# pvjosue/CWFA

Measured on AMD Instinct MI355X. Metric: volumes/sec inverse-pass @512×512×96 fp32; NLL match vs ref (1/2/4/8 GPU), higher is better.
Workload: dtype f32 (storage, accumulation, wavelets, couplings); convolution products on the bf16 matrix cores from an exact three-way bf16 split of both fp32 operands, six products per fp32 product: fp32-equivalent; plain-fp32-MFMA figure: fp32_mfma; 1 GPU; 512x512x96 volume, 4-scale CWFA (CAT blocks, 64 ch) + LRNN inverse, z=0, batch 1/GPU, random-init weights (BASELINE.json configs[2]); precision=split, parallelism=replicated x1 (independent volumes per GPU, no collective)

## Files before the change

cwfa_amd/build.py:

```python
import os
import subprocess
import sys
from concurrent.futures import ThreadPoolExecutor

HERE = os.path.dirname(os.path.abspath(__file__))
CSRC = os.path.join(HERE, "csrc")
INCLUDE = os.path.join(os.path.dirname(HERE), "include")
LIB = os.path.join(HERE, "libcwfa_hip.so")
SOURCES = ["elementwise.hip", "conv2d.hip", "conv_wino.hip", "conv_wino2d.hip", "conv_split_layer.hip", "conv_split_out.hip", "conv_split3x3.hip", "conv3d.hip", "conv3d_split.hip", "lrnn_ops.hip", "conv_bwd.hip", "eval_ops.hip", "prep_ops.hip", "optim_ops.hip", "loss_ops.hip", "deconv_ops.hip", "neuron_ops.hip", "noise_ops.hip", "sparse_ops.hip", "register_ops.hip", "register_views_ops.hip", "register3d_ops.hip", "footprint_ops.hip", "trace_ops.hip", "demix_ops.hip"]
HIPCC = os.environ.get("HIPCC", "/opt/rocm/bin/hipcc")
FLAGS = ["--offload-arch=gfx950", "-O3", "-fPIC", "-std=c++17", "-ffp-contract=off", "-I", INCLUDE, "-I", CSRC,
         "-Wall", "-Wno-unused-function"]


EXTRA = {"conv3d_split.hip": ["-fno-slp-vectorize"], "demix_ops.hip": ["-ffp-contract=off"]}


def _newer(src, dst):
    return not os.path.exists(dst) or os.path.getmtime(src) > os.path.getmtime(dst)


def build_all(force=False, verbose=False):
    deps = [os.path.join(CSRC, "common.h"), os.path.join(CSRC, "conv_internal.h"), os.path.join(CSRC, "conv_split_out_geom.h"), os.path.join(CSRC, "register_internal.h"), os.path.join(INCLUDE, "cwfa_hip.h"),
            os.path.abspath(__file__)]
    objs, jobs = [], []
    for s in SOURCES:
        src, obj = os.path.join(CSRC, s), os.path.join(CSRC, s.replace(".hip", ".o"))
        objs.append(obj)
        if force or _newer(src, obj) or any(_newer(d, obj) for d in deps):
            jobs.append([HIPCC, *FLAGS, *EXTRA.get(s, []), "-c", src, "-o", obj])

    def run(cmd):
        if verbose:
            print(" ".join(cmd), flush=True)
        r = subprocess.run(cmd, capture_output=True, text=True)
        if r.returncode != 0:
            raise RuntimeError(f"hipcc failed: {' '.join(cmd)}\n{r.stdout}\n{r.stderr}")
        return r.stderr

    with ThreadPoolExecutor(max_workers=4) as ex:
        for warn in ex.map(run, jobs):
            if verbose and warn.strip():
                print(warn, file=sys.stderr)
    if jobs or force or not os.path.exists(LIB) or any(_newer(o, LIB) for o in objs):
        run([HIPCC, "--offload-arch=gfx950", "-shared", "-fPIC", "-o", LIB, *objs])
    return LIB


if __name__ == "__main__":
    print(build_all(force="--force" in sys.argv, verbose=True))
```

cwfa_amd/csrc/conv2d.hip:

```cpp
#include "conv_internal.h"

#include <string.h>
#include <type_traits>

namespace {

template <int KS_, int CK_, int MT_, int NT_, int WM_, int WN_, int XV_ = 1>
struct Cfg {
    static constexpr int KS = KS_, CK = CK_, MT = MT_, NT = NT_, WM = WM_, WN = WN_;
    static constexpr int XV = XV_;
    static_assert(XV_ == 1 || (XV_ == 4 && KS_ == 1), "vector staging needs halo-free tiles");
    static constexpr int PAD = KS / 2;
    static constexpr int NTHREADS = 64 * WM * WN;
    static constexpr int CT = 32 * MT * WM;
    static constexpr int TR = NT * WN;
    static constexpr int TC = 32;
    static constexpr int XR = TR + KS - 1;
    static constexpr int XC = TC + KS - 1;
    static constexpr int XS = CK * XR * XC;
    static constexpr int XS_PAD = (XS + 3) & ~3;
    static constexpr int WS = KS * KS * CK * CT;
    static constexpr int XPT = (XS / XV + NTHREADS - 1) / NTHREADS;
    static constexpr int WPT = (WS / 4 + NTHREADS - 1) / NTHREADS;
    static constexpr int BUF = XS_PAD + WS;
// ... 521 lines not shown
    if (rc) return rc;
    hipLaunchKernelGGL((conv2d_mfma_kernel<C, EPI, PRO>), grid, dim3(C::NTHREADS), LDS, stream, p);
    CWFA_LAUNCH_CHECK("cwfa_conv2d_f32");
    return CWFA_OK;
}

template <class C, unsigned ALLOWED, bool PRO>
int launch_sel(const ConvParams& p, int epi, hipStream_t st) {
    if (!(ALLOWED & (1u << epi)) && epi != EPI_NONE_BLK8) epi = EPI_GENERIC;
    switch (epi) {
        case EPI_NONE: if constexpr (ALLOWED & (1u << EPI_NONE)) return launch_epi<C, EPI_NONE, PRO>(p, st); break;
        case EPI_ELU: if constexpr (ALLOWED & (1u << EPI_ELU)) return launch_epi<C, EPI_ELU, PRO>(p, st); break;
        case EPI_RES_ELU: if constexpr (ALLOWED & (1u << EPI_RES_ELU)) return launch_epi<C, EPI_RES_ELU, PRO>(p, st); break;
        case EPI_PRELU: if constexpr (ALLOWED & (1u << EPI_PRELU)) return launch_epi<C, EPI_PRELU, PRO>(p, st); break;
        case EPI_RES_PRELU: if constexpr (ALLOWED & (1u << EPI_RES_PRELU)) return launch_epi<C, EPI_RES_PRELU, PRO>(p, st); break;
        case EPI_GELU_RES: if constexpr (ALLOWED & (1u << EPI_GELU_RES)) return launch_epi<C, EPI_GELU_RES, PRO>(p, st); break;
        case EPI_UP: if constexpr (ALLOWED & (1u << EPI_UP)) return launch_epi<C, EPI_UP, PRO>(p, st); break;
        case EPI_NONE_BLK8:
            if constexpr (ALLOWED & (1u << EPI_NONE_BLK8)) return launch_epi<C, EPI_NONE_BLK8, PRO>(p, st);
            cwfa_set_error("cwfa_conv2d_f32: out_blocked8 is built for the 1x1 kernels with more than 32 output channels");
            return CWFA_E_SHAPE;
        default: break;
    }
    return launch_epi<C, EPI_GENERIC, PRO>(p, st);
}

template <class C, unsigned ALLOWED, unsigned ALLOWED_PRO>
int launch(const ConvParams& p, int epi, hipStream_t st) {
    if (p.o.in_scale || p.o.in_add) return launch_sel<C, ALLOWED_PRO, true>(p, epi, st);
    return launch_sel<C, ALLOWED, false>(p, epi, st);
}

}
int g_cwfa_split_xcd_map = 1;
int g_cwfa_split_rows16 = 1;
extern int g_cwfa_mip3_ablate;
extern int g_cwfa_reg_upsample_stages;
namespace {

int fill_params(ConvParams& p, const char* name, const float* x, const float* w_packed, float* y, int B, int Cin, int H,
                int W, int Cout, int64_t x_bs, int64_t y_bs, const cwfa_conv_opts* opts) {
    CWFA_REQUIRE(B >= 0 && Cin > 0 && Cout > 0 && H >= 0 && W >= 0, CWFA_E_INVAL, "%s: bad size", name);
    if (B == 0 || H == 0 || W == 0) return 1;
    CWFA_REQUIRE(x && w_packed && y, CWFA_E_INVAL, "%s: null pointer", name);
    CWFA_REQUIRE(!opts || !opts->out_sample_stats, CWFA_E_INVAL, "%s: out_sample_stats is a feature of the few-channel cwfa_conv7x7_split_f32", name);
    CWFA_REQUIRE((int64_t)Cin * H * W < (1ll << 30) && (int64_t)Cout * H * W * (p.o.upshuffle2 ? 1 : 1) < (1ll << 30), CWFA_E_SHAPE, "%s: C*H*W exceeds the 32-bit byte offsets of a tile (2^30 elements per image)", name);
    CWFA_REQUIRE(cwfa_aligned16(w_packed), CWFA_E_ALIGN, "%s: packed weights must be 16-byte aligned", name);
    p.x = x; p.wp = w_packed; p.y = y;
    p.B = B; p.Cin = Cin; p.H = H; p.W = W; p.Cout = Cout;
    p.x_bs = x_bs; p.y_bs = y_bs;
    p.products = g_cwfa_operand == CwfaOperand::split3 ? 6 : 1;
    if (opts) p.o = *opts;
    CWFA_REQUIRE(!(p.o.in_scale && !p.o.in_shift), CWFA_E_INVAL, "%s: in_scale without in_shift", name);
    CWFA_REQUIRE(p.o.act >= 0 && p.o.act <= CWFA_ACT_RELU && p.o.act2 >= 0 && p.o.act2 <= CWFA_ACT_RELU, CWFA_E_INVAL,
                 "%s: bad activation", name);
    CWFA_REQUIRE(!((p.o.act == CWFA_ACT_PRELU || p.o.act2 == CWFA_ACT_PRELU) && !p.o.prelu_alpha), CWFA_E_INVAL,
                 "%s: PReLU without prelu_alpha", name);
    return CWFA_OK;
}

typedef Cfg<1, 16, 2, 4, 4, 2> CS;
constexpr int CS_XB = 3 * 2 * 8 * 32 * 16, CS_WB = 3 * 2 * 256 * 16, CS_BUFB = CS_XB + CS_WB;

__device__ __forceinline__ void split3(float v, unsigned short (&o)[3]) {
    const __bf16 a1 = (__bf16)v;
    const float r1 = v - (float)a1;
    const __bf16 a2 = (__bf16)r1;
    const float r2 = r1 - (float)a2;
    const __bf16 a3 = (__bf16)r2;
    o[0] = __builtin_bit_cast(unsigned short, a1);
    o[1] = __builtin_bit_cast(unsigned short, a2);
    o[2] = __builtin_bit_cast(unsigned short, a3);
}

__device__ __forceinline__ unsigned short f16_bits(float v) { return __builtin_bit_cast(unsigned short, (_Float16)v); }

template <bool F16 = false>
__global__ __launch_bounds__(256) void split_input_kernel(const float* __restrict__ x, uint4* __restrict__ ws, int Cin, int CG2,
                                                          int64_t HW, int64_t x_bs, const float* __restrict__ sc,
                                                          const float* __restrict__ sh, int64_t aff_bs,
                                                          const float* __restrict__ add, int64_t add_bs) {
    const int64_t px = (int64_t)blockIdx.x * 256 + threadIdx.x;
    if (px >= HW) return;
    const int cg = blockIdx.y, b = blockIdx.z;
    unsigned short pc[3][8];
#pragma unroll
    for (int j = 0; j < 8; ++j) {
        const int c = cg * 8 + j;
        float v = 0.f;
        if (c < Cin) {
            v = x[(int64_t)b * x_bs + (int64_t)c * HW + px];
            if (sc) v = v * sc[(int64_t)b * aff_bs + c] + sh[(int64_t)b * aff_bs + c];
            if (add) v += add[(int64_t)b * add_bs + (int64_t)c * HW + px];
        }
        if constexpr (F16) {
            pc[0][j] = f16_bits(v);
            continue;
        }
        unsigned short o[3];
        split3(v, o);
        pc[0][j] = o[0]; pc[1][j] = o[1]; pc[2][j] = o[2];
    }
#pragma unroll
    for (int q = 0; q < (F16 ? 1 : 3); ++q) {
        uint4 u;
        u.x = pc[q][0] | ((unsigned)pc[q][1] << 16);
        u.y = pc[q][2] | ((unsigned)pc[q][3] << 16);
        u.z = pc[q][4] | ((unsigned)pc[q][5] << 16);
        u.w = pc[q][6] | ((unsigned)pc[q][7] << 16);
        ws[(((int64_t)b * 3 + q) * CG2 + cg) * HW + px] = u;
    }
}

template <bool F16 = false>
__global__ __launch_bounds__(256) void split_pack_kernel(const float* __restrict__ w, uint4* __restrict__ out, int Cout, int Cin,
                                                         int nchunks, int taps, int transposed, int64_t total) {
    const int64_t i = (int64_t)blockIdx.x * blockDim.x + threadIdx.x;
    if (i >= total) return;
    const int col = (int)(i % 256), h = (int)((i / 256) % 2), tap = (int)((i / 512) % taps);
    const int chunk = (int)((i / (512 * (int64_t)taps)) % nchunks);
    const int ctile = (int)(i / ((int64_t)512 * taps * nchunks));
    const int co = ctile * 256 + col;
    unsigned short pc[3][8];
#pragma unroll
    for (int j = 0; j < 8; ++j) {
        const int ci = chunk * 16 + h * 8 + j;
        float v = 0.f;
        if (co < Cout && ci < Cin)
            v = transposed ? w[((int64_t)ci * (Cout / 4) + (co >> 2)) * 4 + (co & 3)] : w[((int64_t)co * Cin + ci) * taps + tap];
        if constexpr (F16) {
            pc[0][j] = f16_bits(v);
            pc[1][j] = pc[2][j] = 0;
            continue;
        }
        unsigned short o[3];
        split3(v, o);
        pc[0][j] = o[0]; pc[1][j] = o[1]; pc[2][j] = o[2];
    }
#pragma unroll
    for (int q = 0; q < 3; ++q) {
        uint4 u;
        u.x = pc[q][0] | ((unsigned)pc[q][1] << 16);
        u.y = pc[q][2] | ((unsigned)pc[q][3] << 16);
        u.z = pc[q][4] | ((unsigned)pc[q][5] << 16);
        u.w = pc[q][6] | ((unsigned)pc[q][7] << 16);
        out[((((int64_t)ctile * nchunks + chunk) * taps + tap) * 3 + q) * 512 + h * 256 + col] = u;
    }
}

struct SplitParams {
    ConvParams c;
    const void* ws;
    int CG2;
    int64_t ws_bs;
};

template <int EPI, bool F16 = false>
__global__ __launch_bounds__(512, 1) void conv1x1_split_kernel(SplitParams sp) {
    typedef CS C;
    const ConvParams& p = sp.c;
    extern __shared__ __attribute__((aligned(16))) float smem[];
    char* lds = reinterpret_cast<char*>(smem);
    const Tile t = make_tile<C>(p);
    const bool six = p.products != 1;
    const int tid = threadIdx.x, wave = tid >> 6;
    const int64_t HW = (int64_t)p.H * p.W;
    constexpr unsigned OOB = 0x80000000u;

    unsigned xoff[3];
#pragma unroll
    for (int i = 0; i < 3; ++i) {
        const int e = tid + i * 512;
        const int px = e & 31, row = (e >> 5) & 7, h = (e >> 8) & 1, piece = e >> 9;
        const int gr = t.row0 + row, gc = t.col0 + px;
        xoff[i] = (gr < p.H && gc < p.W) ? (unsigned)((((int64_t)piece * sp.CG2 + h) * HW + (int64_t)gr * p.W + gc) * 16) : OOB;
    }
    const auto rx = CWFA_RSRC(reinterpret_cast<const char*>(sp.ws) + (int64_t)t.b * sp.ws_bs, (int)sp.ws_bs);
    const auto rw = CWFA_RSRC(reinterpret_cast<const char*>(p.wp) + (int64_t)t.ct * p.nchunks * CS_WB, p.nchunks * CS_WB);
    const int xchunk = (int)(2 * HW * 16);
    constexpr int NPC = F16 ? 1 : 3;
    auto dma = [&](int chunk, int buf) {
        char* base = lds + buf * CS_BUFB + wave * 1024;
#pragma unroll
        for (int i = 0; i < NPC; ++i)
            __builtin_amdgcn_raw_ptr_buffer_load_lds(rx, (lds_ptr)(base + i * 8192), 16, xoff[i], chunk * xchunk, 0, 0);
#pragma unroll
        for (int i = 0; i < NPC; ++i)
            __builtin_amdgcn_raw_ptr_buffer_load_lds(rw, (lds_ptr)(base + CS_XB + i * 8192), 16, (unsigned)(tid + i * 512) * 16u,
                                                     chunk * CS_WB, 0, 0);
    };

    f32x16 acc[2][4];
#pragma unroll
    for (int m = 0; m < 2; ++m)
#pragma unroll
        for (int n = 0; n < 4; ++n)
#pragma unroll
            for (int r = 0; r < 16; ++r) acc[m][n][r] = 0.f;

    const char* alane = lds + CS_XB + ((t.kh * 256) + t.wm * 64 + t.l31) * 16;
    const char* blane = lds + ((t.kh * 8 + t.wn * 4) * 32 + t.l31) * 16;

    dma(0, 0);
    dma(1, 1);
    if constexpr (F16) asm volatile("s_waitcnt vmcnt(2)" ::: "memory");
    else asm volatile("s_waitcnt vmcnt(6)" ::: "memory");
    __builtin_amdgcn_s_barrier();
    int buf = 0;
    for (int chunk = 0; chunk < p.nchunks; ++chunk) {
        int nb = buf + 2;
        nb = nb >= 3 ? nb - 3 : nb;
        dma(chunk + 2, nb);
        const char* ab = alane + buf * CS_BUFB;
        const char* bb = blane + buf * CS_BUFB;
        bf16x8 A[2][3], Bq[2][3];
#pragma unroll
        for (int m = 0; m < 2; ++m)
#pragma unroll
            for (int q = 0; q < 3; ++q) A[m][q] = *reinterpret_cast<const bf16x8*>(ab + (q * 512 + m * 32) * 16);
#pragma unroll
        for (int q = 0; q < 3; ++q) Bq[0][q] = *reinterpret_cast<const bf16x8*>(bb + (q * 512) * 16);
#pragma unroll
        for (int n = 0; n < 4; ++n) {
            if (n < 3) {
#pragma unroll
                for (int q = 0; q < 3; ++q) Bq[(n + 1) & 1][q] = *reinterpret_cast<const bf16x8*>(bb + (q * 512 + (n + 1) * 32) * 16);
            }
#pragma unroll
            for (int m = 0; m < 2; ++m) {
                f32x16 c = acc[m][n];
                if constexpr (F16) {
                    acc[m][n] = __builtin_amdgcn_mfma_f32_32x32x16_f16(__builtin_bit_cast(f16x8, A[m][0]), __builtin_bit_cast(f16x8, Bq[n & 1][0]),
                                                                       c, 0, 0, 0);
                    continue;
                }
                if (six) {
                    c = __builtin_amdgcn_mfma_f32_32x32x16_bf16(A[m][2], Bq[n & 1][0], c, 0, 0, 0);
                    c = __builtin_amdgcn_mfma_f32_32x32x16_bf16(A[m][1], Bq[n & 1][1], c, 0, 0, 0);
                    c = __builtin_amdgcn_mfma_f32_32x32x16_bf16(A[m][0], Bq[n & 1][2], c, 0, 0, 0);
                    c = __builtin_amdgcn_mfma_f32_32x32x16_bf16(A[m][1], Bq[n & 1][0], c, 0, 0, 0);
                    c = __builtin_amdgcn_mfma_f32_32x32x16_bf16(A[m][0], Bq[n & 1][1], c, 0, 0, 0);
                }
                c = __builtin_amdgcn_mfma_f32_32x32x16_bf16(A[m][0], Bq[n & 1][0], c, 0, 0, 0);
                acc[m][n] = c;
            }
        }
        if constexpr (F16) asm volatile("s_waitcnt vmcnt(2)\n\ts_waitcnt lgkmcnt(0)" ::: "memory");
        else asm volatile("s_waitcnt vmcnt(6)\n\ts_waitcnt lgkmcnt(0)" ::: "memory");
        __builtin_amdgcn_s_barrier();
        buf = buf + 1 == 3 ? 0 : buf + 1;
    }
    asm volatile("s_waitcnt vmcnt(0)" ::: "memory");
    __syncthreads();
    epilogue<C, EPI>(p, t, acc);
}

template <int EPI>
int launch_split(SplitParams sp, hipStream_t stream) {
    ConvParams& p = sp.c;
    p.tiles_x = (p.W + CS::TC - 1) / CS::TC;
    p.tiles_y = (p.H + CS::TR - 1) / CS::TR;
    const int ctiles = (p.Cout + CS::CT - 1) / CS::CT;
    CWFA_REQUIRE((int64_t)p.tiles_x * p.tiles_y < (1ll << 31) && ctiles <= 65535 && p.B <= 65535, CWFA_E_SHAPE,
                 "cwfa_conv_split_f32: grid too large");
    constexpr int LDS = 3 * CS_BUFB;
    return cwfa_with_operand([&](auto, auto f16) -> int {
        constexpr auto kern = &conv1x1_split_kernel<EPI, f16>;
        const int rc = cwfa_max_lds<kern>(LDS, "cwfa_conv_split_f32");
        if (rc) return rc;
        hipLaunchKernelGGL(kern, dim3((unsigned)(p.tiles_x * p.tiles_y), ctiles, p.B), dim3(512), LDS, stream, sp);
        CWFA_LAUNCH_CHECK("cwfa_conv_split_f32");
        return CWFA_OK;
    });
}

}

extern "C" int64_t cwfa_split_workspace_bytes(int B, int Cin, int64_t HW) {
    if (B < 0 || Cin <= 0 || HW < 0) return -1;
    const int64_t CG2 = 2 * ((Cin + 15) / 16);
    return (int64_t)B * 3 * CG2 * HW * 16;
}

extern "C" int cwfa_split_input_f32(const float* x, void* ws, int B, int Cin, int64_t HW, int64_t x_bs, const float* in_scale,
                                    const float* in_shift, int64_t in_affine_bs, const float* in_add, int64_t in_add_bs,
                                    void* stream) {
    CWFA_REQUIRE(x && ws, CWFA_E_INVAL, "cwfa_split_input_f32: null pointer");
    CWFA_REQUIRE(B >= 0 && Cin > 0 && HW >= 0 && B <= 65535, CWFA_E_SHAPE, "cwfa_split_input_f32: bad shape");
    CWFA_REQUIRE(!in_scale == !in_shift, CWFA_E_INVAL, "cwfa_split_input_f32: in_scale and in_shift go together");
    CWFA_REQUIRE(cwfa_aligned16(ws), CWFA_E_ALIGN, "cwfa_split_input_f32: workspace must be 16-byte aligned");
    if (B == 0 || HW == 0) return CWFA_OK;
    const int CG2 = 2 * ((Cin + 15) / 16);
    CWFA_REQUIRE((int64_t)3 * CG2 * HW * 16 < (1ll << 31), CWFA_E_SHAPE, "cwfa_split_input_f32: one sample's planes must stay below 2 GiB");
    return cwfa_with_operand([&](auto, auto f16) -> int {
        hipLaunchKernelGGL(split_input_kernel<f16>, dim3((unsigned)((HW + 255) / 256), CG2, B), dim3(256), 0, (hipStream_t)stream, x,
                           reinterpret_cast<uint4*>(ws), Cin, CG2, HW, x_bs, in_scale, in_shift, in_affine_bs, in_add, in_add_bs);
        CWFA_LAUNCH_CHECK("cwfa_split_input_f32");
        return CWFA_OK;
    });
}

extern "C" int64_t cwfa_conv_split_packed_bytes(int Cout, int Cin, int ks) {
    if (Cout <= 0 || Cin <= 0 || ks != 1) return -1;
    return (int64_t)((Cout + 255) / 256) * ((Cin + 15) / 16) * CS_WB;
}

extern "C" int cwfa_conv_split_pack_f32(const float* w, void* packed, int Cout, int Cin, int ks, int transposed, void* stream) {
    CWFA_REQUIRE(w && packed, CWFA_E_INVAL, "cwfa_conv_split_pack_f32: null pointer");
    CWFA_REQUIRE(Cout > 0 && Cin > 0 && ks == 1 && (!transposed || Cout % 4 == 0), CWFA_E_SHAPE,
                 "cwfa_conv_split_pack_f32: bad shape (1x1 / transposed 2x2 only; 3x3: cwfa_conv3x3_split_pack_f32)");
    CWFA_REQUIRE(cwfa_aligned16(packed), CWFA_E_ALIGN, "cwfa_conv_split_pack_f32: packed image must be 16-byte aligned");
    const int nchunks = (Cin + 15) / 16, taps = ks * ks;
    const int64_t total = (int64_t)((Cout + 255) / 256) * nchunks * taps * 512;
    return cwfa_with_operand([&](auto, auto f16) -> int {
        hipLaunchKernelGGL(split_pack_kernel<f16>, dim3((unsigned)((total + 255) / 256)), dim3(256), 0, (hipStream_t)stream, w,
                           reinterpret_cast<uint4*>(packed), Cout, Cin, nchunks, taps, transposed, total);
        CWFA_LAUNCH_CHECK("cwfa_conv_split_pack_f32");
        return CWFA_OK;
    });
}

extern "C" int cwfa_conv_split_f32(const void* ws, const void* w_packed, float* y, int B, int Cin, int H, int W, int Cout, int ks,
                                   int64_t y_bs, const cwfa_conv_opts* opts, void* stream) {
    CWFA_REQUIRE(!(opts && (opts->in_blocked8 || opts->out_blocked8 || opts->in_cat)), CWFA_E_INVAL,
                 "cwfa_conv_split_f32: blocked layouts / two-source inputs are not built here");
    CWFA_REQUIRE(ws && w_packed && y, CWFA_E_INVAL, "cwfa_conv_split_f32: null pointer");
    CWFA_REQUIRE(ks == 1, CWFA_E_SHAPE, "cwfa_conv_split_f32: kernel size %d (1x1 only; 3x3: cwfa_conv3x3_split_f32)", ks);
    SplitParams sp{};
    int rc = fill_params(sp.c, "cwfa_conv_split_f32", reinterpret_cast<const float*>(ws), reinterpret_cast<const float*>(w_packed), y,
                         B, Cin, H, W, Cout, 0, y_bs, opts);
    if (rc) return rc < 0 ? rc : CWFA_OK;
    ConvParams& p = sp.c;
    CWFA_REQUIRE(!p.o.in_scale && !p.o.in_add, CWFA_E_INVAL, "cwfa_conv_split_f32: the load-side prologue belongs in cwfa_split_input_f32");
    CWFA_REQUIRE(!p.o.upshuffle2 || (ks == 1 && Cout % 4 == 0), CWFA_E_SHAPE, "cwfa_conv_split_f32: upshuffle2 needs ks=1, Cout=4*Co");
    CWFA_REQUIRE(!p.o.out_stats && !p.o.prelu_per_channel, CWFA_E_INVAL, "cwfa_conv_split_f32: out_stats / prelu_per_channel are features of cwfa_conv3x3_split_f32");
    p.nchunks = (Cin + 15) / 16;
    sp.ws = ws;
    sp.CG2 = 2 * p.nchunks;
    sp.ws_bs = (int64_t)3 * sp.CG2 * H * W * 16;
    CWFA_REQUIRE(sp.ws_bs + (int64_t)4 * H * W * 16 < (1ll << 31) && (int64_t)(p.nchunks * ks * ks + 2) * CS_WB < (1ll << 31), CWFA_E_SHAPE,
                 "cwfa_conv_split_f32: one sample's planes / one cout tile's weights must stay below 2 GiB");
    const int epi = classify_epilogue(p.o);
    hipStream_t st = (hipStream_t)stream;
    switch (epi) {
        case EPI_NONE: return launch_split<EPI_NONE>(sp, st);
        case EPI_UP: return launch_split<EPI_UP>(sp, st);
        default: return launch_split<EPI_GENERIC>(sp, st);
    }
}

int g_cwfa_wino_min_cout = 1;
int g_cwfa_wino_2d = 512;
CwfaOperand g_cwfa_operand = CwfaOperand::split3;

extern "C" int cwfa_set_option(const char* name, int value) {
    CWFA_REQUIRE(name, CWFA_E_INVAL, "cwfa_set_option: null name");
    if (strcmp(name, "winograd_min_cout") == 0) {
        g_cwfa_wino_min_cout = value;
        return CWFA_OK;
    }
    if (strcmp(name, "winograd_2d") == 0) {
        g_cwfa_wino_2d = value;
        return CWFA_OK;
    }
    if (strcmp(name, "wgrad_split") == 0) {
        g_cwfa_wgrad_split = value != 0;
        return CWFA_OK;
    }
    if (strcmp(name, "wgrad_rows") == 0) {
        g_cwfa_wgrad_rows = value;
        return CWFA_OK;
    }
    if (strcmp(name, "split3x3_xcd_map") == 0) {
        g_cwfa_split_xcd_map = value;
        return CWFA_OK;
    }
    if (strcmp(name, "mip3_ablate") == 0) {
        CWFA_REQUIRE(value >= 0 && value <= 7, CWFA_E_INVAL, "cwfa_set_option: mip3_ablate is a mask of bits 0..2");
        g_cwfa_mip3_ablate = value;
        return CWFA_OK;
    }
    if (strcmp(name, "reg_upsample_stages") == 0) {
        CWFA_REQUIRE(value >= 0 && value <= 7, CWFA_E_INVAL, "cwfa_set_option: reg_upsample_stages is a mask of bits 0..2");
        g_cwfa_reg_upsample_stages = value;
        return CWFA_OK;
    }
    if (strcmp(name, "split3x3_rows16") == 0) {
        g_cwfa_split_rows16 = value;
        return CWFA_OK;
    }
    if (strcmp(name, "split_products") == 0) {
        CWFA_REQUIRE(value == 1 || value == 6, CWFA_E_INVAL, "cwfa_set_option: split_products must be 1 or 6");
        CWFA_REQUIRE(value == 1 || g_cwfa_operand != CwfaOperand::fp16, CWFA_E_INVAL,
                     "cwfa_set_option: split_products = 6 needs split_operand = 0 (the three-piece split is a bf16 format)");
        if (value == 6) g_cwfa_operand = CwfaOperand::split3;
        else if (g_cwfa_operand == CwfaOperand::split3) g_cwfa_operand = CwfaOperand::bf16;
        return CWFA_OK;
    }
    if (strcmp(name, "split_operand") == 0) {
        CWFA_REQUIRE(value == 0 || value == 1, CWFA_E_INVAL, "cwfa_set_option: split_operand must be 0 (bf16) or 1 (fp16)");
        CWFA_REQUIRE(value == 0 || g_cwfa_operand != CwfaOperand::split3, CWFA_E_INVAL,
                     "cwfa_set_option: split_operand = 1 (fp16) needs split_products = 1 (fp16 operands take one product)");
        if (value == 1) g_cwfa_operand = CwfaOperand::fp16;
        else if (g_cwfa_operand == CwfaOperand::fp16) g_cwfa_operand = CwfaOperand::bf16;
        return CWFA_OK;
    }
    cwfa_set_error("cwfa_set_option: unknown option '%s'", name);
    return CWFA_E_INVAL;
}

extern "C" int64_t cwfa_conv2d_packed_floats(int Cout, int Cin, int ks) {
    const Sel s = select_cfg(ks, Cout);
    if (s.id < 0 || Cout <= 0 || Cin <= 0) return -1;
    if (cwfa_wino_selected(ks, Cout)) return cwfa_wino_packed_floats(Cout, Cin);
    const int64_t ctiles = (Cout + s.CT - 1) / s.CT, nchunks = (Cin + s.CK - 1) / s.CK;
    return ctiles * nchunks * ks * ks * s.CK * s.CT;
}

extern "C" int cwfa_conv2d_pack_f32(const float* w, float* packed, int Cout, int Cin, int ks, int transposed, void* stream) {
    CWFA_REQUIRE(w && packed, CWFA_E_INVAL, "cwfa_conv2d_pack_f32: null pointer");
    CWFA_REQUIRE(!transposed || (ks == 1 && Cout % 4 == 0), CWFA_E_SHAPE,
                 "cwfa_conv2d_pack_f32: transposed source needs ks=1 (2x2 stride-2 deconv as 1x1) and Cout = 4*Co");
    const int64_t total = cwfa_conv2d_packed_floats(Cout, Cin, ks);
    CWFA_REQUIRE(total > 0, CWFA_E_SHAPE, "cwfa_conv2d_pack_f32: unsupported filter %dx%d, Cout=%d, Cin=%d", ks, ks, Cout, Cin);
    if (cwfa_wino_selected(ks, Cout)) return cwfa_wino_pack(w, packed, Cout, Cin, (hipStream_t)stream);
    const Sel s = select_cfg(ks, Cout);
    const int nchunks = (Cin + s.CK - 1) / s.CK;
    hipLaunchKernelGGL(pack_kernel, dim3((unsigned)((total + 255) / 256)), dim3(256), 0, (hipStream_t)stream, w, packed, Cout,
                       Cin, ks, s.CT, s.CK, nchunks, total, transposed);
    CWFA_LAUNCH_CHECK("cwfa_conv2d_pack_f32");
    return CWFA_OK;
}

extern "C" int cwfa_conv2d_f32(const float* x, const float* w_packed, float* y, int B, int Cin, int H, int W, int Cout, int ks,
                               int64_t x_bs, int64_t y_bs, const cwfa_conv_opts* opts, void* stream) {
    CWFA_REQUIRE(!(opts && opts->in_blocked8), CWFA_E_INVAL, "cwfa_conv2d_f32: in_blocked8 is a cwfa_conv3x3_split_f32 feature");
    CWFA_REQUIRE(!(opts && opts->in_cat) || (ks == 1 && Cout <= 64 && !opts->in_scale && !opts->in_add && opts->in_cat_from % 16 == 0 &&
                                             opts->in_cat_from > 0 && opts->in_cat_from < Cin && opts->in_cat_c1 > 0 &&
                                             opts->in_cat_c1 <= opts->in_cat_from),
                 CWFA_E_INVAL, "cwfa_conv2d_f32: in_cat needs a 1x1 bank with <= 64 outputs packed with in_cat_from (a multiple of 16) "
                               "columns for the first source, and no load-side affine / add");
    CWFA_REQUIRE(!(opts && opts->out_blocked8) || (ks == 1 && Cout % 8 == 0 && !opts->residual && opts->act == CWFA_ACT_NONE &&
                                                   opts->act2 == CWFA_ACT_NONE && !opts->upshuffle2 && !opts->in_scale && !opts->in_add &&
                                                   cwfa_aligned16(y) && (y_bs & 3) == 0 && (!opts->bias || cwfa_aligned16(opts->bias))),
                 CWFA_E_INVAL, "cwfa_conv2d_f32: out_blocked8 needs a plain 1x1 bank (bias only), Cout %% 8 == 0 and 16-byte aligned y / bias");
    const Sel s = select_cfg(ks, Cout);
    CWFA_REQUIRE(s.id >= 0, CWFA_E_SHAPE, "cwfa_conv2d_f32: kernel size %d not in {1,3,7}", ks);
    ConvParams p{};
    int rc = fill_params(p, "cwfa_conv2d_f32", x, w_packed, y, B, Cin, H, W, Cout, x_bs, y_bs, opts);
    if (rc) return rc < 0 ? rc : CWFA_OK;
    CWFA_REQUIRE(!p.o.upshuffle2 || (ks == 1 && Cout % 4 == 0), CWFA_E_SHAPE, "cwfa_conv2d_f32: upshuffle2 needs ks=1, Cout=4*Co");
    CWFA_REQUIRE(!p.o.out_stats && !p.o.prelu_per_channel, CWFA_E_INVAL, "cwfa_conv2d_f32: out_stats / prelu_per_channel are features of cwfa_conv3x3_split_f32");
    const int epi = classify_epilogue(p.o);
    hipStream_t st = (hipStream_t)stream;
    if (cwfa_wino_selected(ks, Cout)) return cwfa_wino_conv(x, w_packed, y, B, Cin, H, W, Cout, x_bs, y_bs, p.o, st);
    constexpr unsigned N = 1u << EPI_NONE, E = 1u << EPI_ELU, RE = 1u << EPI_RES_ELU, P = 1u << EPI_PRELU,
                       RP = 1u << EPI_RES_PRELU, G = 1u << EPI_GELU_RES, U = 1u << EPI_UP, K = 1u << EPI_NONE_BLK8;
    const bool v4 = ks == 1 && (W & 3) == 0 && (x_bs & 3) == 0 && (reinterpret_cast<uintptr_t>(x) & 15) == 0 &&
                    (!p.o.in_add || ((p.o.in_add_bs & 3) == 0 && (reinterpret_cast<uintptr_t>(p.o.in_add) & 15) == 0));
    if (v4) {
        switch (s.id) {
            case 3: return launch<C1v_32, N | P | G, P>(p, epi, st);
            case 4: return launch<C1v_64, N | RE | G | K, 0>(p, epi, st);
            default: return launch<C1v_128, N | U | K, U>(p, epi, st);
        }
    }
    switch (s.id) {
        case 0: return launch<C3_32, N | P | RP, 0>(p, epi, st);
        case 1: return launch<C3_64, N | E | P | RP, 0>(p, epi, st);
        case 2: return launch<C3_128, N | P, P>(p, epi, st);
        case 3: return launch<C1_32, N | P | G, P>(p, epi, st);
        case 4: return launch<C1_64, N | RE | G | K, 0>(p, epi, st);
        case 5: return launch<C1_128, N | U | K, U>(p, epi, st);
        case 6: return launch<C7_32, N, 0>(p, epi, st);
        default: return launch<C7_64, N, 0>(p, epi, st);
    }
}

extern "C" int cwfa_subnet_pack1x1_f32(const float* w, float* panel, void* stream) {
    CWFA_REQUIRE(w && panel, CWFA_E_INVAL, "cwfa_subnet_pack1x1_f32: null pointer");
    hipLaunchKernelGGL(pack1x1_kernel, dim3(16), dim3(256), 0, (hipStream_t)stream, w, panel);
    CWFA_LAUNCH_CHECK("cwfa_subnet_pack1x1_f32");
    return CWFA_OK;
}

extern "C" int cwfa_subnet_layer_tape_f32(const float* x, const float* w3_packed, const float* b3, const float* w1_panel,
                                          const float* b1, float* y, float* hidden, int B, int H, int W, int64_t x_bs, int64_t y_bs,
                                          int64_t hidden_bs, void* stream) {
    ConvParams p{};
    cwfa_conv_opts o{};
    o.bias = b3;
    int rc = fill_params(p, "cwfa_subnet_layer_tape_f32", x, w3_packed, y, B, 64, H, W, 64, x_bs, y_bs, &o);
    if (rc) return rc < 0 ? rc : CWFA_OK;
    CWFA_REQUIRE(b3 && w1_panel && b1 && hidden, CWFA_E_INVAL, "cwfa_subnet_layer_tape_f32: null pointer");
    CWFA_REQUIRE(x != y && x != hidden && y != hidden, CWFA_E_INVAL, "cwfa_subnet_layer_tape_f32: x, y and hidden must be distinct");
    CWFA_REQUIRE(cwfa_aligned16(w1_panel), CWFA_E_ALIGN, "cwfa_subnet_layer_tape_f32: 1x1 panel must be 16-byte aligned");
    CWFA_REQUIRE(cwfa_wino_selected(3, 64), CWFA_E_INVAL,
                 "cwfa_subnet_layer_tape_f32: needs the Winograd packing of the 3x3 bank (option winograd_min_cout <= 64)");
    return cwfa_wino_layer(x, w3_packed, b3, w1_panel, b1, y, B, H, W, x_bs, y_bs, (hipStream_t)stream, hidden, hidden_bs);
}

extern "C" int cwfa_subnet_layer_f32(const float* x, const float* w3_packed, const float* b3, const float* w1_panel,
                                     const float* b1, float* y, int B, int H, int W, int64_t x_bs, int64_t y_bs, void* stream) {
    ConvParams p{};
    cwfa_conv_opts o{};
    o.bias = b3;
    int rc = fill_params(p, "cwfa_subnet_layer_f32", x, w3_packed, y, B, 64, H, W, 64, x_bs, y_bs, &o);
    if (rc) return rc < 0 ? rc : CWFA_OK;
    CWFA_REQUIRE(b3 && w1_panel && b1, CWFA_E_INVAL, "cwfa_subnet_layer_f32: null pointer");
    CWFA_REQUIRE(x != y, CWFA_E_INVAL, "cwfa_subnet_layer_f32: in-place not supported (3x3 halo)");
    CWFA_REQUIRE(cwfa_aligned16(w1_panel), CWFA_E_ALIGN, "cwfa_subnet_layer_f32: 1x1 panel must be 16-byte aligned");
    if (cwfa_wino_selected(3, 64))
        return cwfa_wino_layer(x, w3_packed, b3, w1_panel, b1, y, B, H, W, x_bs, y_bs, (hipStream_t)stream);
    static_assert(CL::CT == 64 && C3_64::CT == 64 && C3_64::CK == CL::CK, "fused layer shares the 3x3 64-channel packing");
    p.w1x1 = w1_panel;
    p.b1x1 = b1;
    dim3 grid;
    rc = prepare<CL>(p, grid);
    if (rc) return rc;
    hipLaunchKernelGGL(subnet_layer_kernel, grid, dim3(CL::NTHREADS), CL::LDS_BYTES, (hipStream_t)stream, p);
    CWFA_LAUNCH_CHECK("cwfa_subnet_layer_f32");
    return CWFA_OK;
}
```

cwfa_amd/csrc/conv_internal.h:

```cpp
#pragma once
#include "common.h"
#include <type_traits>

enum class CwfaOperand : int { split3, bf16, fp16 };
extern CwfaOperand g_cwfa_operand;

template <class F>
int cwfa_with_operand(F&& f) {
    switch (g_cwfa_operand) {
        case CwfaOperand::split3: return f(std::true_type{}, std::false_type{});
        case CwfaOperand::bf16: return f(std::false_type{}, std::false_type{});
        case CwfaOperand::fp16: break;
    }
    return f(std::false_type{}, std::true_type{});
}

template <auto KERN>
int cwfa_max_lds(int bytes, const char* entry) {
    static bool done = false;
    if (done) return CWFA_OK;
    const hipError_t e = hipFuncSetAttribute(reinterpret_cast<const void*>(KERN), hipFuncAttributeMaxDynamicSharedMemorySize, bytes);
    if (e != hipSuccess) {
        cwfa_set_error("%s: cannot raise the dynamic LDS limit to %d bytes: %s", entry, bytes, hipGetErrorString(e));
        return CWFA_E_HIP;
    }
    done = true;
    return CWFA_OK;
}

extern int g_cwfa_wino_min_cout;
static inline bool cwfa_wino_selected(int ks, int Cout) { return ks == 3 && Cout >= g_cwfa_wino_min_cout; }

extern int g_cwfa_wgrad_rows;
extern int g_cwfa_wgrad_split;
extern int g_cwfa_wino_2d;
static inline bool cwfa_wino2d_selected(int Cout) { return g_cwfa_wino_2d != 0 && Cout > 64 && Cout >= g_cwfa_wino_2d; }
int64_t cwfa_wino2d_packed_floats(int Cout, int Cin);
int cwfa_wino2d_pack(const float* w, float* packed, int Cout, int Cin, hipStream_t stream);
int cwfa_wino2d_conv(const float* x, const float* w_packed, float* y, int B, int Cin, int H, int W, int Cout, int64_t x_bs,
                     int64_t y_bs, const cwfa_conv_opts& o, hipStream_t stream);

int64_t cwfa_wino_packed_floats(int Cout, int Cin);
int cwfa_wino_pack(const float* w, float* packed, int Cout, int Cin, hipStream_t stream);
int cwfa_wino_conv(const float* x, const float* w_packed, float* y, int B, int Cin, int H, int W, int Cout, int64_t x_bs,
                   int64_t y_bs, const cwfa_conv_opts& o, hipStream_t stream);
int cwfa_wino_layer(const float* x, const float* w3_packed, const float* b3, const float* w1_panel, const float* b1, float* y,
                    int B, int H, int W, int64_t x_bs, int64_t y_bs, hipStream_t stream, float* hidden = nullptr,
                    int64_t hidden_bs = 0);
```

Measured before the change: 57.47 volumes/s.

## Add persistent triple-buffered split-bf16 kernel for transposed 2x2 upsample convs

Transposed 2x2 (upshuffle) 1x1 convolutions now go to a dedicated persistent kernel instead of the generic split kernel's EPI_UP epilogue. Each block loops over tiles and keeps three LDS buffers. Weight and input tiles are DMA'd directly into LDS with buffer_load_lds, overlapped with the six-product MFMA chain, and stepped 32 input channels at a time. The weight pack uses a new layout, so the packed size changes. This adds a new code path and a different weight format, and the kernel's large LDS footprint limits it to one block per CU.

```diff
diff --git a/cwfa_amd/build.py b/cwfa_amd/build.py
--- a/cwfa_amd/build.py
+++ b/cwfa_amd/build.py
@@ -7,7 +7,7 @@
 CSRC = os.path.join(HERE, "csrc")
 INCLUDE = os.path.join(os.path.dirname(HERE), "include")
 LIB = os.path.join(HERE, "libcwfa_hip.so")
-SOURCES = ["elementwise.hip", "conv2d.hip", "conv_wino.hip", "conv_wino2d.hip", "conv_split_layer.hip", "conv_split_out.hip", "conv_split3x3.hip", "conv3d.hip", "conv3d_split.hip", "lrnn_ops.hip", "conv_bwd.hip", "eval_ops.hip", "prep_ops.hip", "optim_ops.hip", "loss_ops.hip", "deconv_ops.hip", "neuron_ops.hip", "noise_ops.hip", "sparse_ops.hip", "register_ops.hip", "register_views_ops.hip", "register3d_ops.hip", "footprint_ops.hip", "trace_ops.hip", "demix_ops.hip"]
+SOURCES = ["elementwise.hip", "conv2d.hip", "conv_split_up.hip", "conv_wino.hip", "conv_wino2d.hip", "conv_split_layer.hip", "conv_split_out.hip", "conv_split3x3.hip", "conv3d.hip", "conv3d_split.hip", "lrnn_ops.hip", "conv_bwd.hip", "eval_ops.hip", "prep_ops.hip", "optim_ops.hip", "loss_ops.hip", "deconv_ops.hip", "neuron_ops.hip", "noise_ops.hip", "sparse_ops.hip", "register_ops.hip", "register_views_ops.hip", "register3d_ops.hip", "footprint_ops.hip", "trace_ops.hip", "demix_ops.hip"]
 HIPCC = os.environ.get("HIPCC", "/opt/rocm/bin/hipcc")
 FLAGS = ["--offload-arch=gfx950", "-O3", "-fPIC", "-std=c++17", "-ffp-contract=off", "-I", INCLUDE, "-I", CSRC,
          "-Wall", "-Wno-unused-function"]
diff --git a/cwfa_amd/csrc/conv2d.hip b/cwfa_amd/csrc/conv2d.hip
--- a/cwfa_amd/csrc/conv2d.hip
+++ b/cwfa_amd/csrc/conv2d.hip
@@ -847,7 +847,8 @@
 
 extern "C" int64_t cwfa_conv_split_packed_bytes(int Cout, int Cin, int ks) {
     if (Cout <= 0 || Cin <= 0 || ks != 1) return -1;
-    return (int64_t)((Cout + 255) / 256) * ((Cin + 15) / 16) * CS_WB;
+    static_assert(CWFA_UP_STEP_BYTES == 2 * CS_WB, "a 32-channel step of the transposed bank is two 16-channel chunks");
+    return cwfa_up_split_packed_bytes(Cout, Cin);
 }
 
 extern "C" int cwfa_conv_split_pack_f32(const float* w, void* packed, int Cout, int Cin, int ks, int transposed, void* stream) {
@@ -855,6 +856,7 @@
     CWFA_REQUIRE(Cout > 0 && Cin > 0 && ks == 1 && (!transposed || Cout % 4 == 0), CWFA_E_SHAPE,
                  "cwfa_conv_split_pack_f32: bad shape (1x1 / transposed 2x2 only; 3x3: cwfa_conv3x3_split_pack_f32)");
     CWFA_REQUIRE(cwfa_aligned16(packed), CWFA_E_ALIGN, "cwfa_conv_split_pack_f32: packed image must be 16-byte aligned");
+    if (transposed) return cwfa_up_split_pack(w, packed, Cout, Cin, (hipStream_t)stream);
     const int nchunks = (Cin + 15) / 16, taps = ks * ks;
     const int64_t total = (int64_t)((Cout + 255) / 256) * nchunks * taps * 512;
     return cwfa_with_operand([&](auto, auto f16) -> int {
@@ -885,13 +887,9 @@
     sp.ws_bs = (int64_t)3 * sp.CG2 * H * W * 16;
     CWFA_REQUIRE(sp.ws_bs + (int64_t)4 * H * W * 16 < (1ll << 31) && (int64_t)(p.nchunks * ks * ks + 2) * CS_WB < (1ll << 31), CWFA_E_SHAPE,
                  "cwfa_conv_split_f32: one sample's planes / one cout tile's weights must stay below 2 GiB");
-    const int epi = classify_epilogue(p.o);
     hipStream_t st = (hipStream_t)stream;
-    switch (epi) {
-        case EPI_NONE: return launch_split<EPI_NONE>(sp, st);
-        case EPI_UP: return launch_split<EPI_UP>(sp, st);
-        default: return launch_split<EPI_GENERIC>(sp, st);
-    }
+    if (p.o.upshuffle2) return cwfa_up_split_conv(ws, w_packed, y, B, Cin, H, W, Cout, sp.CG2, sp.ws_bs, y_bs, p.o, st);
+    return classify_epilogue(p.o) == EPI_NONE ? launch_split<EPI_NONE>(sp, st) : launch_split<EPI_GENERIC>(sp, st);
 }
 
 int g_cwfa_wino_min_cout = 1;
diff --git a/cwfa_amd/csrc/conv_internal.h b/cwfa_amd/csrc/conv_internal.h
--- a/cwfa_amd/csrc/conv_internal.h
+++ b/cwfa_amd/csrc/conv_internal.h
@@ -40,6 +40,12 @@
 int cwfa_wino2d_conv(const float* x, const float* w_packed, float* y, int B, int Cin, int H, int W, int Cout, int64_t x_bs,
                      int64_t y_bs, const cwfa_conv_opts& o, hipStream_t stream);
 
+constexpr int CWFA_UP_STEP_BYTES = 3 * 4 * 256 * 16;
+int64_t cwfa_up_split_packed_bytes(int Cout, int Cin);
+int cwfa_up_split_pack(const float* w, void* packed, int Cout, int Cin, hipStream_t stream);
+int cwfa_up_split_conv(const void* ws, const void* packed, float* y, int B, int Cin, int H, int W, int Cout, int CG2, int64_t ws_bs,
+                       int64_t y_bs, const cwfa_conv_opts& o, hipStream_t stream);
+
 int64_t cwfa_wino_packed_floats(int Cout, int Cin);
 int cwfa_wino_pack(const float* w, float* packed, int Cout, int Cin, hipStream_t stream);
 int cwfa_wino_conv(const float* x, const float* w_packed, float* y, int B, int Cin, int H, int W, int Cout, int64_t x_bs,
diff --git a/cwfa_amd/csrc/conv_split_up.hip b/cwfa_amd/csrc/conv_split_up.hip
--- /dev/null
+++ b/cwfa_amd/csrc/conv_split_up.hip
@@ -0,0 +1,304 @@
+#include "conv_internal.h"
+#include "conv_split_out_geom.h"
+
+extern int g_cwfa_split_xcd_map;
+
+namespace {
+
+constexpr int HALF = CWFA_UP_STEP_BYTES;
+constexpr int UP_LDS = 3 * HALF;
+
+struct UpParams {
+    const char* ws;
+    const char* wp;
+    float* y;
+    const float* bias;
+    const float* residual;
+    const float* prelu_alpha;
+    int act, act2;
+    int B, H, W, Cout, nsteps, CG2, ptiles, rtiles, ntiles, xmap;
+    int64_t ws_bs, y_bs, res_bs;
+};
+
+__device__ __forceinline__ unsigned short up_f16_bits(float v) { return __builtin_bit_cast(unsigned short, (_Float16)v); }
+
+template <bool F16>
+__global__ __launch_bounds__(256) void up_pack_kernel(const float* __restrict__ w, uint4* __restrict__ out, int Cout, int Cin, int nsteps,
+                                                      int64_t total) {
+    const int64_t i = (int64_t)blockIdx.x * blockDim.x + threadIdx.x;
+    if (i >= total) return;
+    const int row = (int)(i % 256), g = (int)((i / 256) % 4), q = (int)((i / 1024) % 3);
+    const int step = (int)((i / 3072) % nsteps), ctile = (int)(i / ((int64_t)3072 * nsteps));
+    const int co = ctile * 256 + row;
+    unsigned short pc[8];
+#pragma unroll
+    for (int j = 0; j < 8; ++j) {
+        const int ci = step * 32 + g * 8 + j;
+        float v = 0.f;
+        if (co < Cout && ci < Cin) v = w[((int64_t)ci * (Cout / 4) + (co >> 2)) * 4 + (co & 3)];
+        if constexpr (F16) {
+            pc[j] = q == 0 ? up_f16_bits(v) : (unsigned short)0;
+        } else {
+            __bf16 a[3];
+            cwfa_split3<true>(v, a[0], a[1], a[2]);
+            pc[j] = __builtin_bit_cast(unsigned short, q == 0 ? a[0] : q == 1 ? a[1] : a[2]);
+        }
+    }
+    uint4 u;
+    u.x = pc[0] | ((unsigned)pc[1] << 16);
+    u.y = pc[2] | ((unsigned)pc[3] << 16);
+    u.z = pc[4] | ((unsigned)pc[5] << 16);
+    u.w = pc[6] | ((unsigned)pc[7] << 16);
+    out[i] = u;
+}
+
+template <bool SIX> constexpr int UP_NPC = SIX ? 3 : 1;
+template <bool SIX> constexpr int UP_ND = 2 * UP_NPC<SIX>;
+
+#define UP_DMA(SRC, BYTES, BASE, VO, SOFF, TAIL)                                                                                 \
+    do {                                                                                                                         \
+        const auto r_ = CWFA_RSRC(SRC, BYTES);                                                                                   \
+        char* b_ = (BASE);                                                                                                       \
+        const bool t_ = (TAIL);                                                                                                  \
+        _Pragma("unroll") for (int i_ = 0; i_ < ND; ++i_)                                                                        \
+            __builtin_amdgcn_raw_ptr_buffer_load_lds(r_, (lds_ptr)(b_ + i_ * 8192), 16, (t_ && (i_ & 1)) ? OOB : (VO)[i_], SOFF, 0, 0); \
+    } while (0)
+
+template <bool SIX, bool F16, bool GEN>
+__global__ __launch_bounds__(512, 1) void upconv_split_kernel(UpParams p) {
+    static_assert(!(SIX && F16), "fp16 operands: single product only");
+    extern __shared__ __attribute__((aligned(16))) char up_smem[];
+    char* lds = up_smem;
+    constexpr int NPC = UP_NPC<SIX>, ND = UP_ND<SIX>;
+    constexpr unsigned OOB = 0x80000000u;
+    const int tid = threadIdx.x, lane = tid & 63, wave = __builtin_amdgcn_readfirstlane(tid >> 6);
+    const int wm = wave >> 1, wn = wave & 1, l15 = lane & 15, kg = lane >> 4;
+    const int HW = p.H * p.W, grid = (int)gridDim.x;
+
+    auto decode = [&](int it, int& b, int& pix0, int& rt) {
+        const int tile = p.xmap ? (it & 7) * (p.ntiles >> 3) + (it >> 3) : it;
+        const int r = tile / p.rtiles;
+        rt = tile - r * p.rtiles;
+        b = r / p.ptiles;
+        pix0 = (r - b * p.ptiles) * 256;
+    };
+
+    int lit = (int)blockIdx.x, lstep = 0;
+    const char *xbase = p.ws, *wbase = p.wp;
+    unsigned xoff[6];
+    auto aim = [&]() {
+        int b, pix0, rt;
+        decode(lit < p.ntiles ? lit : 0, b, pix0, rt);
+        xbase = p.ws + (int64_t)b * p.ws_bs;
+        wbase = p.wp + (int64_t)rt * p.nsteps * HALF;
+#pragma unroll
+        for (int i = 0; i < ND; ++i) {
+            const int e = tid + i * 512;
+            const int gp = pix0 + (e & 255), g = (e >> 8) & 3, q = e >> 10;
+            xoff[i] = gp < HW ? (unsigned)((((int64_t)q * p.CG2 + g) * HW + gp) * 16) : OOB;
+        }
+    };
+    aim();
+    const int xbytes = (int)p.ws_bs, wbytes = p.nsteps * HALF;
+    unsigned woff[6];
+#pragma unroll
+    for (int i = 0; i < ND; ++i) woff[i] = (unsigned)(tid + i * 512) * 16u;
+    auto b_tail = [&]() { return lstep == p.nsteps - 1 && (p.CG2 & 2) != 0; };
+    auto advance = [&]() {
+        if (++lstep < p.nsteps) return;
+        lstep = 0;
+        lit += grid;
+        aim();
+    };
+
+    f32x4 acc[4][8];
+#pragma unroll
+    for (int m = 0; m < 4; ++m)
+#pragma unroll
+        for (int n = 0; n < 8; ++n) acc[m][n] = f32x4{0.f, 0.f, 0.f, 0.f};
+
+    const char* afrag = lds + (kg * 256 + wm * 64 + l15) * 16;
+    const char* bfrag = lds + (kg * 256 + wn * 128 + l15) * 16;
+
+    UP_DMA(wbase, wbytes, lds + wave * 1024, woff, 0, false);
+    UP_DMA(xbase, xbytes, lds + HALF + wave * 1024, xoff, 0, b_tail());
+    advance();
+    asm volatile("s_waitcnt vmcnt(0)" ::: "memory");
+    __builtin_amdgcn_s_barrier();
+    int sa = 0;
+    for (int it = (int)blockIdx.x; it < p.ntiles; it += grid) {
+        for (int step = 0; step < p.nsteps; ++step) {
+            const int sb = sa == 2 ? 0 : sa + 1, sc = sb == 2 ? 0 : sb + 1;
+            const bool more = lit < p.ntiles;
+            if (more) UP_DMA(wbase, wbytes, lds + sc * HALF + wave * 1024, woff, lstep * HALF, false);
+            const char* ab = afrag + sa * HALF;
+            const char* bb = bfrag + sb * HALF;
+            bf16x8 A[4][NPC], Bq[2][NPC];
+#pragma unroll
+            for (int m = 0; m < 4; ++m)
+#pragma unroll
+                for (int q = 0; q < NPC; ++q) A[m][q] = *reinterpret_cast<const bf16x8*>(ab + (q * 1024 + m * 16) * 16);
+#pragma unroll
+            for (int q = 0; q < NPC; ++q) Bq[0][q] = *reinterpret_cast<const bf16x8*>(bb + (q * 1024) * 16);
+#pragma unroll
+            for (int n = 0; n < 8; ++n) {
+                if (n < 7) {
+#pragma unroll
+                    for (int q = 0; q < NPC; ++q) Bq[(n + 1) & 1][q] = *reinterpret_cast<const bf16x8*>(bb + (q * 1024 + (n + 1) * 16) * 16);
+                }
+                CWFA_FENCE();
+#pragma unroll
+                for (int m = 0; m < 4; ++m) {
+                    f32x4 c = acc[m][n];
+                    if constexpr (SIX) {
+                        CWFA_MFMA(A[m][2], Bq[n & 1][0], c);
+                        CWFA_MFMA(A[m][1], Bq[n & 1][1], c);
+                        CWFA_MFMA(A[m][0], Bq[n & 1][2], c);
+                        CWFA_MFMA(A[m][1], Bq[n & 1][0], c);
+                        CWFA_MFMA(A[m][0], Bq[n & 1][1], c);
+                    }
+                    CWFA_MFMA_OP(F16, A[m][0], Bq[n & 1][0], c);
+                    acc[m][n] = c;
+                }
+                CWFA_FENCE();
+                if (n == 0) {
+                    asm volatile("s_waitcnt lgkmcnt(0)" ::: "memory");
+                    __builtin_amdgcn_s_barrier();
+                    if (more) {
+                        UP_DMA(xbase, xbytes, lds + sa * HALF + wave * 1024, xoff, lstep * (4 * HW * 16), b_tail());
+                        advance();
+                    }
+                }
+            }
+            asm volatile("s_waitcnt vmcnt(0)\n\ts_waitcnt lgkmcnt(0)" ::: "memory");
+            __builtin_amdgcn_s_barrier();
+            sa = sc;
+        }
+
+        int b, pix0, rt;
+        decode(it, b, pix0, rt);
+        float* yb = p.y + (int64_t)b * p.y_bs;
+        const int W2 = 2 * p.W;
+        const bool al = (p.y_bs & 1) == 0 && (reinterpret_cast<uintptr_t>(p.y) & 7) == 0;
+        int off[8];
+#pragma unroll
+        for (int n = 0; n < 8; ++n) {
+            const int px = pix0 + wn * 128 + n * 16 + l15;
+            const int row = px / p.W, col = px - row * p.W;
+            off[n] = px < HW ? 2 * row * W2 + 2 * col : -1;
+        }
+        const int c0 = rt * 64 + wm * 16 + kg, Co = p.Cout >> 2;
+        if constexpr (!GEN) {
+#pragma unroll
+            for (int m = 0; m < 4; ++m) {
+                const int c = c0 + m * 4;
+                if (c < Co) {
+                    const float bias = p.bias ? p.bias[c] : 0.f;
+                    float* yc = yb + (int64_t)c * (4 * (int64_t)HW);
+#pragma unroll
+                    for (int n = 0; n < 8; ++n) {
+                        if (off[n] < 0) continue;
+                        float* o = yc + off[n];
+                        const f32x4 v = acc[m][n] + bias;
+                        if (al) {
+                            *reinterpret_cast<float2*>(o) = make_float2(v[0], v[1]);
+                            *reinterpret_cast<float2*>(o + W2) = make_float2(v[2], v[3]);
+                        } else {
+                            o[0] = v[0]; o[1] = v[1]; o[W2] = v[2]; o[W2 + 1] = v[3];
+                        }
+                    }
+                }
+            }
+        } else {
+            const float alpha = (p.prelu_alpha && (p.act == CWFA_ACT_PRELU || p.act2 == CWFA_ACT_PRELU)) ? *p.prelu_alpha : 0.f;
+            const float* rb = p.residual ? p.residual + (int64_t)b * p.res_bs : nullptr;
+#pragma unroll 1
+            for (int mn = 0; mn < 32; ++mn) {
+                f32x4 v = f32x4{0.f, 0.f, 0.f, 0.f};
+                int o_ = -1;
+#pragma unroll
+                for (int k = 0; k < 32; ++k)
+                    if (k == mn) {
+                        v = acc[k >> 3][k & 7];
+                        o_ = off[k & 7];
+                    }
+                const int c = c0 + (mn >> 3) * 4;
+                if (c >= Co || o_ < 0) continue;
+                const float bias = p.bias ? p.bias[c] : 0.f;
+                const int64_t o = (int64_t)c * (4 * (int64_t)HW) + o_;
+                const int64_t os[4] = {o, o + 1, o + W2, o + W2 + 1};
+#pragma unroll
+                for (int r = 0; r < 4; ++r) {
+                    float t = cwfa_act(v[r] + bias, p.act, alpha);
+                    if (rb) t += rb[os[r]];
+                    yb[os[r]] = cwfa_act(t, p.act2, alpha);
+                }
+            }
+        }
+#pragma unroll
+        for (int m = 0; m < 4; ++m)
+#pragma unroll
+            for (int n = 0; n < 8; ++n) acc[m][n] = f32x4{0.f, 0.f, 0.f, 0.f};
+    }
+}
+
+int g_up_cus = 0;
+
+template <bool SIX, bool F16, bool GEN>
+int up_launch(const UpParams& p, int grid, hipStream_t st) {
+    constexpr auto kern = &upconv_split_kernel<SIX, F16, GEN>;
+    const int rc = cwfa_max_lds<kern>(UP_LDS, "cwfa_conv_split_f32");
+    if (rc) return rc;
+    hipLaunchKernelGGL(kern, dim3(grid), dim3(512), UP_LDS, st, p);
+    CWFA_LAUNCH_CHECK("cwfa_conv_split_f32");
+    return CWFA_OK;
+}
+
+}
+
+int64_t cwfa_up_split_packed_bytes(int Cout, int Cin) { return (int64_t)((Cout + 255) / 256) * ((Cin + 31) / 32) * HALF; }
+
+int cwfa_up_split_pack(const float* w, void* packed, int Cout, int Cin, hipStream_t stream) {
+    const int nsteps = (Cin + 31) / 32;
+    const int64_t total = (int64_t)((Cout + 255) / 256) * nsteps * 3072;
+    return cwfa_with_operand([&](auto, auto f16) -> int {
+        hipLaunchKernelGGL(up_pack_kernel<f16>, dim3((unsigned)((total + 255) / 256)), dim3(256), 0, stream, w,
+                           reinterpret_cast<uint4*>(packed), Cout, Cin, nsteps, total);
+        CWFA_LAUNCH_CHECK("cwfa_conv_split_pack_f32");
+        return CWFA_OK;
+    });
+}
+
+int cwfa_up_split_conv(const void* ws, const void* packed, float* y, int B, int Cin, int H, int W, int Cout, int CG2, int64_t ws_bs,
+                       int64_t y_bs, const cwfa_conv_opts& o, hipStream_t stream) {
+    UpParams p{};
+    p.ws = reinterpret_cast<const char*>(ws);
+    p.wp = reinterpret_cast<const char*>(packed);
+    p.y = y;
+    p.bias = o.bias; p.residual = o.residual; p.prelu_alpha = o.prelu_alpha;
+    p.act = o.act; p.act2 = o.act2; p.res_bs = o.res_bs;
+    p.B = B; p.H = H; p.W = W; p.Cout = Cout;
+    p.nsteps = (Cin + 31) / 32;
+    p.CG2 = CG2; p.ws_bs = ws_bs; p.y_bs = y_bs;
+    const int64_t HW = (int64_t)H * W;
+    p.ptiles = (int)((HW + 255) / 256);
+    p.rtiles = (Cout + 255) / 256;
+    const int64_t ntiles = (int64_t)B * p.ptiles * p.rtiles;
+    CWFA_REQUIRE(ntiles < (1ll << 30) && ws_bs + (2 * HW + 256) * 16 < (1ll << 31) && (int64_t)p.nsteps * HALF < (1ll << 31), CWFA_E_SHAPE,
+                 "cwfa_conv_split_f32: one sample's planes / one cout tile's weights must stay below 2 GiB");
+    p.ntiles = (int)ntiles;
+    if (g_up_cus == 0) {
+        int dev = 0, n = 0;
+        if (hipGetDevice(&dev) != hipSuccess || hipDeviceGetAttribute(&n, hipDeviceAttributeMultiprocessorCount, dev) != hipSuccess || n <= 0) {
+            cwfa_set_error("cwfa_conv_split_f32: cannot query the CU count");
+            return CWFA_E_HIP;
+        }
+        g_up_cus = n;
+    }
+    const int grid = cwfa_out::grid_of(ntiles, g_up_cus);
+    p.xmap = cwfa_out::xcd_walk(g_cwfa_split_xcd_map, p.ntiles, grid) ? 1 : 0;
+    const bool gen = o.residual || o.act != CWFA_ACT_NONE || o.act2 != CWFA_ACT_NONE;
+    return cwfa_with_operand([&](auto six, auto f16) -> int {
+        return gen ? up_launch<six, f16, true>(p, grid, stream) : up_launch<six, f16, false>(p, grid, stream);
+    });
+}
```

After: 57.77 volumes/s, median of 6. No clear change (+0.5%).
